# JuliaDSP/DSP.jl

Hardware: AMD Instinct MI355X
Metric: Gsamples/s filt+welch, 1 Gsample Float32 stream; achieved HBM GB/s vs roofline (higher is better)
Workload: dtype f32; 1 GPU; filt(256 taps, overlap-save nfft 2048) + welch_pgram(nfft 4096, hanning, 50 %) per 2^30-sample Float32 stream; one stream per GPU; RCCL all-reduce of the PSD for N>1; samples_per_gpu=1073741824, engine=fused, collective=none (1 GPU), collective_check=not run (--full checks it)

## Files before the change

dsp.jl_amd/_lib.py:

```python
from __future__ import annotations

import ctypes as C
import os
import threading

HERE = os.path.dirname(os.path.abspath(__file__))
LIB_PATH = os.path.join(HERE, "libmi355dsp" + ("_" + os.environ["MDSP_LIB_TAG"] if os.environ.get("MDSP_LIB_TAG") else "") + ".so")

OK, ERR_ARGUMENT, ERR_DOMAIN, ERR_DIMENSION, ERR_ASSERTION, ERR_UNSUPPORTED, ERR_DEVICE, ERR_NOMEM = 0, -1, -2, -3, -4, -5, -6, -7
F32, F64, C32, C64 = 0, 1, 2, 3
ENGINE_AUTO, ENGINE_FUSED, ENGINE_ROCFFT = 0, 1, 2
OLS_FILT, OLS_CONV = 0, 1
HOST_PINNED = 1
COMM_ID_BYTES = 128


class ArgumentError(ValueError):
    """Julia ``ArgumentError``."""


class DomainError(ValueError):
    """Julia ``DomainError``."""


# ... 43 lines not shown
    "mdsp_ols_geometry_for": (ci, [i64, i64, i64, ci, ci, ci, pi64, pi64, pint, pint, pint]),
    "mdsp_ols_exec": (ci, [vp, vp, i64, i64, i64, vp, i64, i64, vp]),
    "mdsp_ols_exec_range": (ci, [vp, vp, i64, i64, i64, vp, i64, i64, i64, vp]),
    "mdsp_ols_exec_host": (ci, [vp, vp, i64, i64, i64, vp, i64, i64, ci]),
    "mdsp_ols_segment": (ci, [vp, vp, i64, i64, i64, vp, vp]),
    "mdsp_frames": (ci, [vp, i64, ci, i64, i64, i64, pdbl, i64, i64, vp, vp]),
    "mdsp_welch_plan_create": (ci, [pvp, i64, i64, i64, pdbl, cd, ci, ci, ci]),
    "mdsp_welch_plan_destroy": (ci, [vp]),
    "mdsp_welch_plan_info": (ci, [vp, pi64, pint]),
    "mdsp_welch_exec": (ci, [vp, vp, i64, i64, i64, vp, i64, vp]),
    "mdsp_welch_reset": (ci, [vp]),
    "mdsp_welch_accumulate": (ci, [vp, vp, i64, i64, i64, vp]),
    "mdsp_welch_frames_accumulated": (ci, [vp, pi64]),
    "mdsp_welch_finalize": (ci, [vp, i64, vp, i64, vp]),
    "mdsp_welch_accumulator": (ci, [vp, pvp, pi64]),
    "mdsp_welch_exec_host": (ci, [vp, vp, i64, i64, i64, vp, i64, ci]),
    "mdsp_comm_unique_id": (ci, [vp]),
    "mdsp_comm_init_rank": (ci, [pvp, vp, ci, ci]),
    "mdsp_comm_destroy": (ci, [vp]),
    "mdsp_comm_info": (ci, [vp, pint, pint]),
    "mdsp_allreduce_sum": (ci, [vp, vp, i64, ci, vp]),
    "mdsp_welch_mean_allreduce": (ci, [vp, vp, i64, i64, i64, vp, vp, vp]),
    "mdsp_welch_allreduce": (ci, [vp, vp, vp]),
    "mdsp_host_alloc": (ci, [pvp, C.c_size_t]),
    "mdsp_host_free": (ci, [vp]),
    "mdsp_host_register": (ci, [vp, C.c_size_t]),
    "mdsp_host_unregister": (ci, [vp]),
    "mdsp_channel_sum": (ci, [vp, i64, i64, i64, ci, vp, vp]),
    "mdsp_stft_plan_create": (ci, [pvp, i64, i64, i64, pdbl, cd, ci, ci, ci, ci]),
    "mdsp_stft_plan_destroy": (ci, [vp]),
# ... 138 lines not shown
```

dsp.jl_amd/csrc/spectral.hip:

```cpp
#include <algorithm>
#include <atomic>
#include <cstdlib>

#include <map>
#include <memory>
#include <mutex>
#include <vector>

#include "common.h"
#include "devio.h"
#include "fft_lds.h"
#include "fft_wg.h"
#include "hostfft.h"
#include "rocfft_wrap.h"
#include "welch_plan.h"
#include "hostpipe.h"
#include "gx_kernels.h"

using namespace mdsp;
using mdsp::fft::cx;

namespace {

inline int64_t rocfft_chunk_bytes() {
// ... 938 lines not shown
            for (int e = 0; e < E; ++e) accp[e] = fft::lanefma(v[e], v[e], accp[e]);
            if (++since == FLUSH) flush();
        } else {
#pragma unroll
            for (int e = 0; e < E; ++e) acc[e] += (double)(v[e].x * v[e].x + v[e].y * v[e].y);
        }
    }
    if constexpr (PAIR) {
        flush();
    } else {
#pragma unroll
        for (int e = 0; e < E; ++e) part[t + T * e] = acc[e];
    }
}

template <int N>
__global__ __launch_bounds__(N / 16, 2) void welch_half3_kernel(SpecArgs a) {
    using R = float;
    constexpr int E = 16, H = 8, PADSHIFT = 5;
    using C = fft::Cfg<N, E>;
    constexpr int T = C::T;
    static_assert(T % 64 == 0 && T >= 128, "one transform per workgroup");
    constexpr int NTWA = C::NTW > 0 ? C::NTW : 1;
    constexpr int REGION = fft::wg_lds_elems<C, PADSHIFT, 1>();
    __shared__ __attribute__((aligned(16))) cx<R> lds[REGION];
    const int t = threadIdx.x;
    const cx<R>* table = static_cast<const cx<R>*>(a.table);
    const int64_t ch = blockIdx.y;

    cx<R> tw[NTWA];
    fft::load_twiddles<C, R, 1, fft::TW_REG>(tw, t, table);
    cx<R> wp[H];
    {
        double wd[E];
        load_window_regs<E, T>(wd, a.win, a.n, t);
#pragma unroll
        for (int e = 0; e < H; ++e) wp[e] = {(R)wd[e], (R)wd[e + H]};
    }
    constexpr int FLUSH = 128;
    cx<R> accp[E];
#pragma unroll
    for (int e = 0; e < E; ++e) accp[e] = {(R)0, (R)0};
    double* part = static_cast<double*>(a.out) + ((int64_t)blockIdx.x * a.nch + ch) * N;
    const __amdgpu_buffer_rsrc_t prs = io::make_rsrc(part, (int64_t)N * 8);
    int since = 0;
    bool first = true;
    auto flush = [&]() {
        int off = t * 8;
        asm volatile("" : "+v"(off));
        if (first) {
#pragma unroll
            for (int e = 0; e < E; ++e) io::Ld<double>::store((double)accp[e].x + (double)accp[e].y, prs, off + T * e * 8);
        } else {
#pragma unroll
            for (int e = 0; e < E; ++e) {
                const double s = io::Ld<double>::load(prs, off + T * e * 8) + ((double)accp[e].x + (double)accp[e].y);
                io::Ld<double>::store(s, prs, off + T * e * 8);
            }
        }
#pragma unroll
        for (int e = 0; e < E; ++e) accp[e] = {(R)0, (R)0};
        first = false;
        since = 0;
    };

    const R* sc = static_cast<const R*>(a.s) + ch * a.lds_;
    const int64_t nslots = (int64_t)gridDim.x;
    int64_t wbase = (int64_t)blockIdx.x * a.run_len, wj = 0;
    auto unit_cur = [&](bool more) { return (more && wbase + wj < a.units_per_ch) ? wbase + wj : a.units_per_ch; };
    auto walk = [&]() {
        if (++wj == a.run_len) {
            wj = 0;
            wbase += nslots * a.run_len;
        }
    };
    auto half_rsrc = [&](int64_t u, int h, bool on) {
        const int64_t pos = u * N + (int64_t)h * (N / 2);
        return io::make_rsrc(sc + pos, on ? std::min<int64_t>(N / 2, a.len - pos) * 4 : 0);
    };
    auto ld8 = [&](cx<R> (&dst)[H], bool to_x, const __amdgpu_buffer_rsrc_t r) {
        int off = t * 4;
        asm volatile("" : "+v"(off));
#pragma unroll
// ... 81 lines not shown
#else
        fft::pass0_windowed<C, PADSHIFT>(Q, F, wp, t, lds);
#endif
        const bool carry = unext == u + 1 && unext < a.units_per_ch;
        load_unit(F, Q, !xa, unext, carry);
        u = unext;
        tail();
    };
    for (int64_t it = 0; it < a.niter; it += 2) {
        unit(P1, P2, true, it + 1 < a.niter);
        if (it + 1 < a.niter) unit(P2, P1, false, it + 2 < a.niter);
    }
    flush();
#ifdef MDSP_WELCH_PROF
    if (a.rinv && (threadIdx.x & 63) == 0) {
        unsigned long long* rec = (unsigned long long*)a.rinv + ((size_t)blockIdx.x * (T / 64) + threadIdx.x / 64) * 16;
        for (int k = 0; k < 13; ++k) rec[k] = prof_sum[k];
        rec[13] = prof_units;
        rec[14] = prof_last - prof_t0;
    }
#undef MDSP_STAMP
#endif
}

template <int N> int welch_run_half3(mdsp_welch_plan_s* pl, SpecArgs& a, hipStream_t st, int* nslices) {
    auto kern = welch_half3_kernel<N>;
    constexpr int threads = N / 16;
    int grid = 1;
    MDSP_TRY(grid_for(kern, threads, a.units_per_ch, a.nch, &grid));
    MDSP_TRY(pl->partial.reserve(sizeof(double) * (size_t)grid * (size_t)a.nch * N));
    a.out = pl->partial.p;
    set_schedule(a, a.units_per_ch, (int64_t)grid);
#ifdef MDSP_WELCH_PROF
    static DevBuf profbuf;
    const size_t nrec = (size_t)grid * (threads / 64);
    MDSP_TRY(profbuf.reserve(nrec * 16 * 8));
    a.rinv = a.nch == 1 ? static_cast<const double*>(profbuf.p) : nullptr;
// ... 19 lines not shown
            totmax = std::max(totmax, (double)h[r * 16 + 14]);
        }
        static const char* nm[13] = {"flush+loop", "load-issue", "barrier1", "reload1", "barrier2", "pass1+ldsW", "barrier3", "reload2", "barrier4", "pass2+acc",
                                     "memwait", "pass0-valu", "pass0-ldsW"};
        fprintf(stderr, "WELCHPROF grid %d x %d waves, %.4f ms, %.0f units/wave, clocks/unit %.0f (max-wave total %.0f clocks -> %.3f GHz):", grid, threads / 64, ms,
                units / nrec, tot / units, totmax, totmax / (ms * 1e6));
        for (int k : {10, 11, 12, 1, 2, 3, 4, 5, 6, 7, 8, 9, 0}) fprintf(stderr, " %s %.0f", nm[k], sum[k] / units);
        fprintf(stderr, "\n");
    }
    (void)hipEventDestroy(e0); (void)hipEventDestroy(e1);
#endif
    *nslices = grid;
    return MDSP_OK;
}

#include "welch_w64.h"

template <typename R, int N, int E, int G, int TWMODE, int PADSHIFT, int NBUF>
int welch_run_half(mdsp_welch_plan_s* pl, SpecArgs& a, hipStream_t st, int* nslices) {
    auto kern = welch_half_kernel<R, N, E, G, TWMODE, PADSHIFT, NBUF>;
    constexpr int threads = (N / E) * G;
    int grid = 1;
    MDSP_TRY(grid_for(kern, threads, cdiv(a.units_per_ch, G), a.nch, &grid));
    MDSP_TRY(pl->partial.reserve(sizeof(double) * (size_t)grid * G * (size_t)a.nch * N));
    a.out = pl->partial.p;
    set_schedule(a, a.units_per_ch, (int64_t)grid * G);
    hipLaunchKernelGGL(kern, dim3(grid, (unsigned)a.nch), dim3(threads), 0, st, a);
    MDSP_LAUNCH_CHECK();
    *nslices = grid * G;
    return MDSP_OK;
// ... 54 lines not shown
    } else {
        bool done = false;
        if constexpr (CPLX && sizeof(R) == 4 && Gm::E > 4) {
            constexpr int T = N / Gm::E;
            const int shift = (!MDSP_DBG(stft_noshift) && a.n == N && a.hop % T == 0 && a.hop / T < Gm::E) ? (int)(a.hop / T) : 0;
            done = shift == 1 || shift == 2 || shift == 4;
            if (shift == 1) rc = welch_run_fused<R, N, Gm::E, Gm::G, Gm::TWREG, pad_default<R>(), CPLX, Gm::NBUF, false, 1>(pl, a, st, &nslices);
            else if (shift == 2) rc = welch_run_fused<R, N, Gm::E, Gm::G, Gm::TWREG, pad_default<R>(), CPLX, Gm::NBUF, false, 2>(pl, a, st, &nslices);
            else if (shift == 4) rc = welch_run_fused<R, N, Gm::E, Gm::G, Gm::TWREG, pad_default<R>(), CPLX, Gm::NBUF, false, 4>(pl, a, st, &nslices);
        }
        if (!done) rc = welch_run_fused<R, N, Gm::E, Gm::G, Gm::TWREG, pad_default<R>(), CPLX, Gm::NBUF, sizeof(R) == 8>(pl, a, st, &nslices);
    }
finalize:
    if (rc != MDSP_OK) return rc;
    MDSP_TRY(pl->reduced.reserve(sizeof(double) * (size_t)a.nch * N));
    MDSP_TRY(reduce_partials(pl, pl->partial.as<double>(), pl->reduced.as<double>(), nslices, a.nch, N, pl->acc_fresh ? 0 : 1, st));
reduced_done:
    if (rc != MDSP_OK) return rc;
    set_fused_sums(pl);
    return MDSP_OK;
}

template <typename R, bool CPLX>
int welch_accumulate_fused(mdsp_welch_plan_s* pl, const void* s, int64_t len, int64_t nch, int64_t lds_, hipStream_t st) {
    const int64_t K = mdsp_frame_count(len, pl->n, pl->noverlap), hop = pl->n - pl->noverlap, N = pl->nfft;
    const double* win = pl->have_win ? pl->win.as<double>() : nullptr;
    if (pl->route != MDSP_ROUTE_POW2 || K == 0) MDSP_TRY(pl->reduced.reserve(sizeof(double) * (size_t)nch * (size_t)N));
    if (K == 0) {
        if (pl->acc_fresh) {
            MDSP_HIP(hipMemsetAsync(pl->reduced.p, 0, sizeof(double) * (size_t)nch * (size_t)N, st));
            set_fused_sums(pl);
// ... 51 lines not shown
            MDSP_TRY(ctcols_welch(pl->ctcols, pl->dtype, s, lds_, K, hop, nch, (int)pl->n, N, pl->r0, win, st, &ngroups, &pl->partial));
            break;
        case MDSP_ROUTE_CTROWS:
            MDSP_TRY(ctrows_welch(pl->ctrows, pl->dtype, pl->r0, s, lds_, K, hop, nch, (int)pl->n, N, win, pl->reduced.as<double>(), pl->acc_fresh, st));
            set_fused_sums(pl);
            return MDSP_OK;
        case MDSP_ROUTE_BIG: {
            using TT = std::conditional_t<CPLX, cx<R>, R>;
            for (int64_t c = 0; c < nch; ++c)
                MDSP_TRY(big::welch(pl->big, pl->dtype, pl->n, N, static_cast<const TT*>(s) + c * lds_, K, hop, win, pl->reduced.as<double>() + c * N, pl->acc_fresh, st));
            set_fused_sums(pl);
            return MDSP_OK;
        }
        default: MDSP_FAIL(MDSP_ERR_ASSERTION, "Welch plan with route %d on the fused engine", pl->route);
    }
    MDSP_TRY(reduce_partials(pl, pl->partial.as<double>(), pl->reduced.as<double>(), (int)ngroups, nch, (int)N, pl->acc_fresh ? 0 : 1, st));
    set_fused_sums(pl);
    return MDSP_OK;
}

}

namespace mdsp {
int gx_run(int id, const GxArgs& a, unsigned grid_x, unsigned grid_y, int threads, size_t lds_bytes, hipStream_t st) {
    switch (id) {
#define MDSP_GX_CASE(ID) case ID: return gx_run_##ID(a, grid_x, grid_y, threads, lds_bytes, st);
        MDSP_GX_CASE(0) MDSP_GX_CASE(1) MDSP_GX_CASE(2) MDSP_GX_CASE(3) MDSP_GX_CASE(5) MDSP_GX_CASE(6) MDSP_GX_CASE(7) MDSP_GX_CASE(8)
        MDSP_GX_CASE(10) MDSP_GX_CASE(11) MDSP_GX_CASE(12) MDSP_GX_CASE(14) MDSP_GX_CASE(15) MDSP_GX_CASE(16) MDSP_GX_CASE(17) MDSP_GX_CASE(19)
#undef MDSP_GX_CASE
        default: MDSP_FAIL(MDSP_ERR_ASSERTION, "gx kernel id %d", id);
    }
// ... 85 lines not shown
    return MDSP_OK;
}

static int welch_check_args(mdsp_welch_plan plan, const void* s_dev, int64_t len, int64_t nch, int64_t lds_) {
    if (!plan) MDSP_FAIL(MDSP_ERR_ARGUMENT, "plan is NULL");
    if (len < 0 || nch < 0) MDSP_FAIL(MDSP_ERR_ARGUMENT, "negative size");
    if (!s_dev && len > 0 && nch > 0) MDSP_FAIL(MDSP_ERR_ARGUMENT, "s is NULL");
    if (nch > 1 && lds_ < len) MDSP_FAIL(MDSP_ERR_DIMENSION, "leading dimension smaller than the column length");
    if (nch > 65535) MDSP_FAIL(MDSP_ERR_UNSUPPORTED, "more than 65535 channels per call");
    return MDSP_OK;
}

int mdsp_welch_reset(mdsp_welch_plan plan) {
    if (!plan) MDSP_FAIL(MDSP_ERR_ARGUMENT, "plan is NULL");
    plan->acc_fresh = true;
    plan->acc_frames = 0;
    plan->acc_nch = 0;
    plan->frames_on_device = false;
    plan->sums_global = false;
    return MDSP_OK;
}

int mdsp_welch_accumulate(mdsp_welch_plan plan, const void* s_dev, int64_t len, int64_t nch, int64_t lds_, void* stream) {
    MDSP_TRY(welch_check_args(plan, s_dev, len, nch, lds_));
    if (nch == 0) return MDSP_OK;
    if (!plan->acc_fresh && plan->acc_nch != nch)
        MDSP_FAIL(MDSP_ERR_DIMENSION, "accumulating %lld channels into sums of %lld channels (mdsp_welch_reset first)", (long long)nch, (long long)plan->acc_nch);
    if (plan->sums_global)
        MDSP_FAIL(MDSP_ERR_ARGUMENT, "these sums are totals over ranks (mdsp_welch_allreduce ran): mdsp_welch_reset before accumulating again");
    hipStream_t st = as_stream(stream);
// ... 21 lines not shown
        MDSP_HIP(hipStreamSynchronize(plan->count_stream));
        MDSP_HIP(hipMemcpy(&k, plan->kdev.p, sizeof(double), hipMemcpyDeviceToHost));
        *frames_per_channel = (int64_t)k;
    }
    return MDSP_OK;
}

int mdsp_welch_accumulator(mdsp_welch_plan plan, void** acc_dev, int64_t* count) {
    if (!plan || !acc_dev || !count) MDSP_FAIL(MDSP_ERR_ARGUMENT, "NULL argument");
    if (plan->acc_fresh) MDSP_FAIL(MDSP_ERR_ARGUMENT, "nothing accumulated since the last mdsp_welch_reset");
    *acc_dev = plan->acc_ptr();
    *count = (int64_t)plan->acc_nslices * plan->acc_nch * plan->acc_nacc;
    return MDSP_OK;
}

int mdsp_welch_finalize(mdsp_welch_plan plan, int64_t frames_total, void* psd_dev, int64_t ldp, void* stream) {
    if (!plan) MDSP_FAIL(MDSP_ERR_ARGUMENT, "plan is NULL");
    if (!psd_dev) MDSP_FAIL(MDSP_ERR_ARGUMENT, "out is NULL");
    if (plan->acc_fresh) MDSP_FAIL(MDSP_ERR_ARGUMENT, "nothing accumulated since the last mdsp_welch_reset");
    if (plan->acc_nch > 1 && ldp < plan->nout) MDSP_FAIL(MDSP_ERR_DIMENSION, "leading dimension smaller than the column length");
    const int64_t K = frames_total > 0 ? frames_total : (plan->frames_on_device ? 0 : plan->acc_frames);
    return dtype_is_double(plan->dtype) ? welch_finalize<double>(plan, K, plan->acc_nch, psd_dev, ldp, as_stream(stream))
                                        : welch_finalize<float>(plan, K, plan->acc_nch, psd_dev, ldp, as_stream(stream));
}

int mdsp_welch_exec(mdsp_welch_plan plan, const void* s_dev, int64_t len, int64_t nch, int64_t lds_, void* psd_dev, int64_t ldp, void* stream) {
    MDSP_TRY(welch_check_args(plan, s_dev, len, nch, lds_));
    if (nch == 0) return MDSP_OK;
    if (!psd_dev) MDSP_FAIL(MDSP_ERR_ARGUMENT, "out is NULL");
    if (nch > 1 && ldp < plan->nout) MDSP_FAIL(MDSP_ERR_DIMENSION, "leading dimension smaller than the column length");
    MDSP_TRY(mdsp_welch_reset(plan));
    MDSP_TRY(mdsp_welch_accumulate(plan, s_dev, len, nch, lds_, stream));
    return mdsp_welch_finalize(plan, 0, psd_dev, ldp, stream);
}

}

template <typename R>
__global__ __launch_bounds__(256) void channel_sum_kernel(const R* __restrict__ psd, R* __restrict__ out, int64_t nout, int64_t nch, int64_t ldp, double scale) {
    const int64_t j = (int64_t)blockIdx.x * blockDim.x + threadIdx.x;
    if (j >= nout) return;
    double a = 0;
    for (int64_t c = 0; c < nch; ++c) a += (double)psd[c * ldp + j];
    const R sum = (R)a;
    out[j] = scale == 1.0 ? sum : (R)((double)sum * scale);
}

// ... 659 lines not shown
```

dsp.jl_amd/csrc/welch_plan.h:

```cpp
#pragma once

#include "common.h"
#include "rocfft_wrap.h"
#include "bigfft.h"
#include "gx_plan.h"
#include "spectral_ctcols.h"
#include "spectral_ctrows.h"

struct mdsp_welch_plan_s {
    int dtype = MDSP_F32, engine = MDSP_ENGINE_ROCFFT, onesided = 1;
    int route = MDSP_ROUTE_ROCFFT, r0 = 0;
    int64_t n = 0, noverlap = 0, nfft = 0, nout = 0;
    double r = 1;
    bool have_win = false;
    mdsp::DevBuf win, table, partial, reduced;
    mdsp::RocPlan fwd;
    mdsp::DevBuf fr, spec;
    int64_t batch = 0;
    int variant = 0;
    bool acc_fresh = true;
    int64_t acc_nch = 0, acc_frames = 0;
    mdsp::DevBuf kdev;
    mdsp::DevBuf redtmp;
    mdsp::big::EngineHolder big;
    mdsp::GxPlan gx;
    mdsp::DevBuf winr;
    bool winr_ready = false;
    mdsp::CtRowsPlan ctrows;
    mdsp::CtColsPlan ctcols;
    mdsp::DevBuf w64prep;
    bool frames_on_device = false;
    bool sums_global = false;
    hipStream_t count_stream = nullptr;
    int acc_nslices = 1, acc_nacc = 0, acc_mode = 0;
    double* acc_ptr() const { return engine == MDSP_ENGINE_ROCFFT ? partial.as<double>() : reduced.as<double>(); }
};
```

dsp.jl_amd/csrc/welch_w64.h:

```cpp
#pragma once

namespace w64 {

constexpr int N = 4096, HALF = N / 2;

#include "welch_w64c_asm_co.h"
#include "welch_w64d_asm_co.h"

struct W64AsmArgs {
    const float* s;
    float* part;
    const float* winpairs;
    const float* tw;
    int64_t lds_, units, run_len, nch;
    int nflush, pad;
};
static_assert(sizeof(W64AsmArgs) == 72, "kernarg layout of mdsp_welch_w64_asm");

__global__ __launch_bounds__(256) void w64asm_prepare_kernel(const double* __restrict__ win, int n, const cx<float>* __restrict__ table, float* __restrict__ out) {
    const int i = blockIdx.x * blockDim.x + threadIdx.x;
    if (i < HALF) {
        out[2 * i] = (float)(i < n ? (win ? win[i] : 1.0) : 0.0);
        out[2 * i + 1] = (float)((i + HALF) < n ? (win ? win[i + HALF] : 1.0) : 0.0);
    }
// ... 7 lines not shown
            tw[14 + 2 * (j - 1) + 1] = b.y;
        }
        for (int k1 = 0; k1 < 4; ++k1) {
            const int m = i + 64 * k1;
            const int e[4] = {m, 2 * m, 4 * m, m + N / 8};
            for (int q = 0; q < 4; ++q) {
                const cx<float> w = table[e[q] & (N - 1)];
                out[2 * HALF + 28 * 64 + 128 * (4 * k1 + q) + 2 * i] = w.x;
                out[2 * HALF + 28 * 64 + 128 * (4 * k1 + q) + 2 * i + 1] = w.y;
            }
        }
    }
}

constexpr int W64_RED_GROUPS = 128;
__global__ __launch_bounds__(256) void w64asm_reduce1_kernel(const float* __restrict__ part, double* __restrict__ tmp, int nslots, int nflush, int64_t nch, int rows_per_group,
                                                             int64_t units, int64_t run_len) {
    const int k4 = (blockIdx.x * 256 + threadIdx.x) * 4;
    const int g = blockIdx.y;
    const int64_t ch = blockIdx.z;
    const int rows = nslots * nflush;
    const int r0 = g * rows_per_group, r1 = min(rows, r0 + rows_per_group);
    double a0 = 0, a1 = 0, a2 = 0, a3 = 0;
#pragma unroll 4
    for (int r = r0; r < r1; ++r) {
        const int sl = r / nflush, f = r - sl * nflush;
        const int64_t mine = min(run_len, units - (int64_t)sl * run_len);
        float4 v = make_float4(0.f, 0.f, 0.f, 0.f);
        if ((int64_t)f * 128 < mine) v = *reinterpret_cast<const float4*>(part + (((int64_t)sl * nch + ch) * nflush + f) * N + k4);
        a0 += (double)v.x;
        a1 += (double)v.y;
        a2 += (double)v.z;
        a3 += (double)v.w;
    }
    double* o = tmp + ((int64_t)ch * W64_RED_GROUPS + g) * N + k4;
    o[0] = a0;
    o[1] = a1;
    o[2] = a2;
    o[3] = a3;
}
__global__ __launch_bounds__(256) void w64asm_reduce2_kernel(const double* __restrict__ tmp, double* __restrict__ reduced, int ngroups, int accumulate) {
    __shared__ double sm[8][32];
    const int b = threadIdx.x & 31, gl = threadIdx.x >> 5;
    const int k = blockIdx.x * 32 + b;
    const int64_t ch = blockIdx.y;
    double t = 0;
    for (int g = gl; g < ngroups; g += 8) t += tmp[((int64_t)ch * W64_RED_GROUPS + g) * N + k];
    sm[gl][b] = t;
    __syncthreads();
    if (gl == 0) {
        t = sm[0][b];
#pragma unroll
        for (int i = 1; i < 8; ++i) t += sm[i][b];
        reduced[ch * N + k] = accumulate ? reduced[ch * N + k] + t : t;
    }
}

struct W64AsmModule {
    hipModule_t mod = nullptr;
    hipFunction_t fn = nullptr;
};
inline int w64asm_function(hipFunction_t* fn, int variant) {
    if (variant != 43 && variant != 44) MDSP_FAIL(MDSP_ERR_ARGUMENT, "no hand-allocated Welch kernel for variant %d", variant);
    static std::mutex mu;
    static W64AsmModule mods[2][64];
    int dev = 0;
    MDSP_HIP(hipGetDevice(&dev));
    std::lock_guard<std::mutex> lk(mu);
    W64AsmModule& m = mods[variant - 43][dev & 63];
    if (!m.fn) {
        MDSP_HIP(hipModuleLoadData(&m.mod, variant == 44 ? welch_w64d_asm_co : welch_w64c_asm_co));
// ... 3 lines not shown
    return MDSP_OK;
}

template <int DUMMY = 0> int welch_run_w64asm(mdsp_welch_plan_s* pl, SpecArgs& a, hipStream_t st, bool* handled, int variant = 44) {
    *handled = false;
    hipFunction_t fn = nullptr;
    MDSP_TRY(w64asm_function(&fn, variant));
    constexpr size_t PREP_FLOATS = 2 * HALF + 28 * 64 + 16 * 128;
    if (pl->w64prep.bytes == 0) {
        MDSP_TRY(pl->w64prep.reserve(PREP_FLOATS * sizeof(float)));
        hipLaunchKernelGGL(w64asm_prepare_kernel, dim3(HALF / 256), dim3(256), 0, st, a.win, a.n, static_cast<const cx<float>*>(a.table), pl->w64prep.as<float>());
        MDSP_LAUNCH_CHECK();
    }
    const int64_t units = a.K / 2;
    MDSP_TRY(pl->reduced.reserve(sizeof(double) * (size_t)a.nch * N));
    bool fresh = pl->acc_fresh;
    if (units > 0) {
        const int64_t per_ch = std::max<int64_t>(1, (int64_t)device_cu_count() / std::max<int64_t>(1, a.nch));
        const int grid = (int)std::max<int64_t>(1, std::min<int64_t>(cdiv(units, 8), per_ch));
        const int64_t nslots = (int64_t)grid * 8;
        const int64_t run_len = cdiv(units, nslots);
        const int nflush = (int)cdiv(run_len, 128);
        const size_t part_bytes = sizeof(float) * (size_t)nslots * (size_t)a.nch * (size_t)nflush * N;
        const size_t tmp_bytes = sizeof(double) * (size_t)a.nch * W64_RED_GROUPS * N;
        MDSP_TRY(pl->partial.reserve(part_bytes + tmp_bytes));
        W64AsmArgs ka;
        ka.s = static_cast<const float*>(a.s);
        ka.part = pl->partial.as<float>();
        ka.winpairs = pl->w64prep.as<float>();
        ka.tw = pl->w64prep.as<float>() + 2 * HALF;
        ka.lds_ = a.lds_;
        ka.units = units;
        ka.run_len = run_len;
        ka.nch = a.nch;
        ka.nflush = nflush;
        ka.pad = 0;
        size_t ksz = sizeof(ka);
        void* cfg[] = {HIP_LAUNCH_PARAM_BUFFER_POINTER, &ka, HIP_LAUNCH_PARAM_BUFFER_SIZE, &ksz, HIP_LAUNCH_PARAM_END};
        MDSP_HIP(hipModuleLaunchKernel(fn, (unsigned)grid, (unsigned)a.nch, 1, 512, 1, 1, 0, st, nullptr, cfg));
        {
            const int rows = (int)nslots * nflush;
            const int rpg = (int)cdiv(rows, W64_RED_GROUPS), ngroups = (int)cdiv(rows, rpg);
            double* tmp = reinterpret_cast<double*>(static_cast<char*>(pl->partial.p) + part_bytes);
            hipLaunchKernelGGL(w64asm_reduce1_kernel, dim3(N / 1024, (unsigned)ngroups, (unsigned)a.nch), dim3(256), 0, st, pl->partial.as<float>(), tmp, (int)nslots, nflush,
                               a.nch, rpg, units, run_len);
            MDSP_LAUNCH_CHECK();
            hipLaunchKernelGGL(w64asm_reduce2_kernel, dim3(N / 32, (unsigned)a.nch), dim3(256), 0, st, tmp, pl->reduced.as<double>(), ngroups, fresh ? 0 : 1);
            MDSP_LAUNCH_CHECK();
        }
        fresh = false;
    }
    if (a.K & 1) {
        SpecArgs t = a;
        t.s = static_cast<const float*>(a.s) + (a.K - 1) * a.hop;
        t.len = a.n;
        t.K = 1;
        t.units_per_ch = 1;
        int ns2 = 0;
        MDSP_TRY((welch_run_half3<N>(pl, t, st, &ns2)));
        hipLaunchKernelGGL(reduce_partials_kernel, dim3((unsigned)cdiv(N, 32), (unsigned)a.nch), dim3(256), 0, st, pl->partial.as<double>(), pl->reduced.as<double>(), ns2,
                           a.nch, N, fresh ? 0 : 1);
        MDSP_LAUNCH_CHECK();
        fresh = false;
    }
    *handled = true;
    return MDSP_OK;
}

}
```

include/mi355dsp.h:

```cpp
#ifndef MI355DSP_H
#define MI355DSP_H

#include <stddef.h>
#include <stdint.h>

#ifdef __cplusplus
extern "C" {
#endif

#define MDSP_VERSION 100

enum {
    MDSP_OK = 0,
    MDSP_ERR_ARGUMENT = -1,
    MDSP_ERR_DOMAIN = -2,
    MDSP_ERR_DIMENSION = -3,
    MDSP_ERR_ASSERTION = -4,
    MDSP_ERR_UNSUPPORTED = -5,
    MDSP_ERR_DEVICE = -6,
    MDSP_ERR_NOMEM = -7
};

enum { MDSP_F32 = 0, MDSP_F64 = 1, MDSP_C32 = 2 , MDSP_C64 = 3  };

// ... 50 lines not shown
                const double* window_host , int64_t first, int64_t count, void* frames_dev,
                void* stream);

typedef struct mdsp_welch_plan_s* mdsp_welch_plan;
int mdsp_welch_plan_create(mdsp_welch_plan* plan, int64_t n, int64_t noverlap, int64_t nfft,
                           const double* window_host, double r, int onesided, int dtype, int engine);
int mdsp_welch_plan_destroy(mdsp_welch_plan plan);
int mdsp_welch_plan_info(mdsp_welch_plan plan, int64_t* nout, int* engine_used);
int mdsp_welch_exec(mdsp_welch_plan plan, const void* s_dev, int64_t len, int64_t nch, int64_t lds,
                    void* psd_dev, int64_t ldp, void* stream);
int mdsp_welch_reset(mdsp_welch_plan plan);
int mdsp_welch_accumulate(mdsp_welch_plan plan, const void* s_dev, int64_t len, int64_t nch, int64_t lds, void* stream);
int mdsp_welch_frames_accumulated(mdsp_welch_plan plan, int64_t* frames_per_channel);
int mdsp_welch_finalize(mdsp_welch_plan plan, int64_t frames_total, void* psd_dev, int64_t ldp, void* stream);
int mdsp_welch_accumulator(mdsp_welch_plan plan, void** acc_dev, int64_t* count);
int mdsp_channel_sum(const void* psd_dev, int64_t nout, int64_t nch, int64_t ldp, int real_dtype, void* sum_dev,
                     void* stream);

#define MDSP_COMM_ID_BYTES 128
typedef struct mdsp_comm_s* mdsp_comm;
int mdsp_comm_unique_id(void* id128 );
int mdsp_comm_init_rank(mdsp_comm* comm, const void* id128, int rank, int nranks);
int mdsp_comm_destroy(mdsp_comm comm);
int mdsp_comm_info(mdsp_comm comm, int* rank, int* nranks);
int mdsp_allreduce_sum(mdsp_comm comm, void* buf_dev, int64_t count, int real_dtype, void* stream);
int mdsp_welch_mean_allreduce(mdsp_welch_plan plan, const void* psd_dev, int64_t nch_local, int64_t ldp, int64_t nch_total,
                              void* mean_dev, mdsp_comm comm, void* stream);
int mdsp_welch_allreduce(mdsp_welch_plan plan, mdsp_comm comm, void* stream);

#define MDSP_HOST_PINNED 1
// ... 148 lines not shown
```

Before: 359.3 Gsamples/s.

## Fuse Welch partial reduction, odd-frame tail and PSD finalize into one kernel

Replaces the two-kernel partial reduction (plus a separate odd-frame half3 launch and reduce) with a single tail kernel. The kernel does a group reduction and uses per-block atomic counters so the last-arriving workgroup performs the final sum and writes the scaled PSD directly. This skips the separate finalize launch when welch_exec is used. The aim is to cut kernel launches and tail latency after the main streaming pass, at the cost of atomic last-block synchronisation and more complex LDS sharing, including running the odd frame inside the tail kernel.

```diff
diff --git a/dsp.jl_amd/_lib.py b/dsp.jl_amd/_lib.py
--- a/dsp.jl_amd/_lib.py
+++ b/dsp.jl_amd/_lib.py
@@ -81,6 +81,7 @@
     "mdsp_welch_frames_accumulated": (ci, [vp, pi64]),
     "mdsp_welch_finalize": (ci, [vp, i64, vp, i64, vp]),
     "mdsp_welch_accumulator": (ci, [vp, pvp, pi64]),
+    "mdsp_welch_rows_reduced": (ci, [vp, pi64]),
     "mdsp_welch_exec_host": (ci, [vp, vp, i64, i64, i64, vp, i64, ci]),
     "mdsp_comm_unique_id": (ci, [vp]),
     "mdsp_comm_init_rank": (ci, [pvp, vp, ci, ci]),
diff --git a/dsp.jl_amd/csrc/spectral.hip b/dsp.jl_amd/csrc/spectral.hip
--- a/dsp.jl_amd/csrc/spectral.hip
+++ b/dsp.jl_amd/csrc/spectral.hip
@@ -976,19 +976,17 @@
     }
 }
 
+template <int N> constexpr int welch_half3_lds() { return fft::wg_lds_elems<fft::Cfg<N, 16>, 5, 1>(); }
 template <int N>
-__global__ __launch_bounds__(N / 16, 2) void welch_half3_kernel(SpecArgs a) {
+__device__ __forceinline__ void welch_half3_units(const SpecArgs& a, cx<float>* lds, const int slot, const int nslots_, const int64_t ch) {
     using R = float;
     constexpr int E = 16, H = 8, PADSHIFT = 5;
     using C = fft::Cfg<N, E>;
     constexpr int T = C::T;
     static_assert(T % 64 == 0 && T >= 128, "one transform per workgroup");
     constexpr int NTWA = C::NTW > 0 ? C::NTW : 1;
-    constexpr int REGION = fft::wg_lds_elems<C, PADSHIFT, 1>();
-    __shared__ __attribute__((aligned(16))) cx<R> lds[REGION];
     const int t = threadIdx.x;
     const cx<R>* table = static_cast<const cx<R>*>(a.table);
-    const int64_t ch = blockIdx.y;
 
     cx<R> tw[NTWA];
     fft::load_twiddles<C, R, 1, fft::TW_REG>(tw, t, table);
@@ -1003,7 +1001,7 @@
     cx<R> accp[E];
 #pragma unroll
     for (int e = 0; e < E; ++e) accp[e] = {(R)0, (R)0};
-    double* part = static_cast<double*>(a.out) + ((int64_t)blockIdx.x * a.nch + ch) * N;
+    double* part = static_cast<double*>(a.out) + ((int64_t)slot * a.nch + ch) * N;
     const __amdgpu_buffer_rsrc_t prs = io::make_rsrc(part, (int64_t)N * 8);
     int since = 0;
     bool first = true;
@@ -1027,8 +1025,8 @@
     };
 
     const R* sc = static_cast<const R*>(a.s) + ch * a.lds_;
-    const int64_t nslots = (int64_t)gridDim.x;
-    int64_t wbase = (int64_t)blockIdx.x * a.run_len, wj = 0;
+    const int64_t nslots = (int64_t)nslots_;
+    int64_t wbase = (int64_t)slot * a.run_len, wj = 0;
     auto unit_cur = [&](bool more) { return (more && wbase + wj < a.units_per_ch) ? wbase + wj : a.units_per_ch; };
     auto walk = [&]() {
         if (++wj == a.run_len) {
@@ -1140,13 +1138,19 @@
     flush();
 #ifdef MDSP_WELCH_PROF
     if (a.rinv && (threadIdx.x & 63) == 0) {
-        unsigned long long* rec = (unsigned long long*)a.rinv + ((size_t)blockIdx.x * (T / 64) + threadIdx.x / 64) * 16;
+        unsigned long long* rec = (unsigned long long*)a.rinv + ((size_t)slot * (T / 64) + threadIdx.x / 64) * 16;
         for (int k = 0; k < 13; ++k) rec[k] = prof_sum[k];
         rec[13] = prof_units;
         rec[14] = prof_last - prof_t0;
     }
 #undef MDSP_STAMP
 #endif
+}
+
+template <int N>
+__global__ __launch_bounds__(N / 16, 2) void welch_half3_kernel(SpecArgs a) {
+    __shared__ __attribute__((aligned(16))) cx<float> lds[welch_half3_lds<N>()];
+    welch_half3_units<N>(a, lds, (int)blockIdx.x, (int)gridDim.x, (int64_t)blockIdx.y);
 }
 
 template <int N> int welch_run_half3(mdsp_welch_plan_s* pl, SpecArgs& a, hipStream_t st, int* nslices) {
@@ -1196,6 +1200,7 @@
     return MDSP_OK;
 }
 
+#include "welch_tail.h"
 #include "welch_w64.h"
 
 template <typename R, int N, int E, int G, int TWMODE, int PADSHIFT, int NBUF>
@@ -1280,7 +1285,9 @@
 finalize:
     if (rc != MDSP_OK) return rc;
     MDSP_TRY(pl->reduced.reserve(sizeof(double) * (size_t)a.nch * N));
-    MDSP_TRY(reduce_partials(pl, pl->partial.as<double>(), pl->reduced.as<double>(), nslices, a.nch, N, pl->acc_fresh ? 0 : 1, st));
+    pl->rows_reduced = nslices;
+    if (pl->fin_psd) MDSP_TRY(tail::run_rows<R>(pl, nslices, a.nch, N, a.K, st));
+    else MDSP_TRY(reduce_partials(pl, pl->partial.as<double>(), pl->reduced.as<double>(), nslices, a.nch, N, pl->acc_fresh ? 0 : 1, st));
 reduced_done:
     if (rc != MDSP_OK) return rc;
     set_fused_sums(pl);
@@ -1362,7 +1369,9 @@
         }
         default: MDSP_FAIL(MDSP_ERR_ASSERTION, "Welch plan with route %d on the fused engine", pl->route);
     }
-    MDSP_TRY(reduce_partials(pl, pl->partial.as<double>(), pl->reduced.as<double>(), (int)ngroups, nch, (int)N, pl->acc_fresh ? 0 : 1, st));
+    pl->rows_reduced = ngroups;
+    if (pl->fin_psd) MDSP_TRY(tail::run_rows<R>(pl, (int)ngroups, nch, (int)N, K, st));
+    else MDSP_TRY(reduce_partials(pl, pl->partial.as<double>(), pl->reduced.as<double>(), (int)ngroups, nch, (int)N, pl->acc_fresh ? 0 : 1, st));
     set_fused_sums(pl);
     return MDSP_OK;
 }
@@ -1478,6 +1487,7 @@
 int mdsp_welch_reset(mdsp_welch_plan plan) {
     if (!plan) MDSP_FAIL(MDSP_ERR_ARGUMENT, "plan is NULL");
     plan->acc_fresh = true;
+    plan->rows_reduced = 0;
     plan->acc_frames = 0;
     plan->acc_nch = 0;
     plan->frames_on_device = false;
@@ -1529,6 +1539,12 @@
     return MDSP_OK;
 }
 
+int mdsp_welch_rows_reduced(mdsp_welch_plan plan, int64_t* rows) {
+    if (!plan || !rows) MDSP_FAIL(MDSP_ERR_ARGUMENT, "NULL argument");
+    *rows = plan->rows_reduced;
+    return MDSP_OK;
+}
+
 int mdsp_welch_finalize(mdsp_welch_plan plan, int64_t frames_total, void* psd_dev, int64_t ldp, void* stream) {
     if (!plan) MDSP_FAIL(MDSP_ERR_ARGUMENT, "plan is NULL");
     if (!psd_dev) MDSP_FAIL(MDSP_ERR_ARGUMENT, "out is NULL");
@@ -1545,7 +1561,12 @@
     if (!psd_dev) MDSP_FAIL(MDSP_ERR_ARGUMENT, "out is NULL");
     if (nch > 1 && ldp < plan->nout) MDSP_FAIL(MDSP_ERR_DIMENSION, "leading dimension smaller than the column length");
     MDSP_TRY(mdsp_welch_reset(plan));
-    MDSP_TRY(mdsp_welch_accumulate(plan, s_dev, len, nch, lds_, stream));
+    plan->fin_psd = plan->engine == MDSP_ENGINE_ROCFFT ? nullptr : psd_dev;
+    plan->fin_ldp = ldp;
+    plan->fin_done = false;
+    const int rc = mdsp_welch_accumulate(plan, s_dev, len, nch, lds_, stream);
+    plan->fin_psd = nullptr;
+    if (rc != MDSP_OK || plan->fin_done) return rc;
     return mdsp_welch_finalize(plan, 0, psd_dev, ldp, stream);
 }
 
diff --git a/dsp.jl_amd/csrc/welch_plan.h b/dsp.jl_amd/csrc/welch_plan.h
--- a/dsp.jl_amd/csrc/welch_plan.h
+++ b/dsp.jl_amd/csrc/welch_plan.h
@@ -28,6 +28,11 @@
     bool winr_ready = false;
     mdsp::CtRowsPlan ctrows;
     mdsp::CtColsPlan ctcols;
+    mdsp::DevBuf tailcnt;
+    void* fin_psd = nullptr;
+    int64_t fin_ldp = 0;
+    bool fin_done = false;
+    int64_t rows_reduced = 0;
     mdsp::DevBuf w64prep;
     bool frames_on_device = false;
     bool sums_global = false;
diff --git a/dsp.jl_amd/csrc/welch_tail.h b/dsp.jl_amd/csrc/welch_tail.h
--- /dev/null
+++ b/dsp.jl_amd/csrc/welch_tail.h
@@ -0,0 +1,279 @@
+#pragma once
+
+namespace tail {
+
+struct TailArgs {
+    const void* rows;
+    double* tmp;
+    double* reduced;
+    const double* odd;
+    void* psd;
+    unsigned* counters;
+    int64_t ldp, nch;
+    int N, nrows, per_group, ngroups;
+    int accumulate, mode, nout, has_odd;
+    double r_total;
+    int nslots, nflush;
+    int64_t units, run_len;
+};
+
+template <int SL> __device__ __forceinline__ int slot_bin(int N, int b, int q) {
+    constexpr int PB = SL / 2;
+    const int p = b * PB + (q < PB ? q : SL - 1 - q);
+    if (p >= (N + 1) / 2) return -1;
+    if (q < PB) return p;
+    if (p == 0) return (N & 1) ? -1 : N / 2;
+    return N - p;
+}
+
+struct __attribute__((packed, aligned(4))) Float4U {
+    float x, y, z, w;
+};
+
+template <int SL> constexpr int lds_sums() { return 8 * SL * 8; }
+template <int SL> constexpr int lds_flags() { return lds_sums<SL>() + SL * 8; }
+constexpr int MAX_FLAGS = 64;
+constexpr int W64_GPW = 4;
+
+template <typename RowT, typename R, int SL>
+__device__ __forceinline__ void phase2(const TailArgs& a, char* smem, const int b, const int NB, const int64_t ch) {
+    constexpr int PB = SL / 2;
+    constexpr bool W64 = sizeof(RowT) == 4;
+    double* sm = reinterpret_cast<double*>(smem);
+    double* fin = reinterpret_cast<double*>(smem + lds_sums<SL>());
+    const int tid = threadIdx.x, N = a.N;
+    const int nsum = a.ngroups > 0 ? a.ngroups : (W64 ? 0 : a.nrows);
+    const double* grp = a.tmp + ((int64_t)ch * NB + b) * a.ngroups * SL;
+    for (int q0 = 0; q0 < SL; q0 += 32) {
+        const int q = q0 + (tid & 31), gl = tid >> 5;
+        const int bin = slot_bin<SL>(N, b, q);
+        double t = 0;
+        if (bin >= 0) {
+            if (a.ngroups > 0) {
+#pragma unroll 4
+                for (int g = gl; g < nsum; g += 8) t += grp[(int64_t)g * SL + q];
+            } else if constexpr (!W64) {
+                const double* rows = static_cast<const double*>(a.rows);
+#pragma unroll 4
+                for (int s = gl; s < nsum; s += 8) t += rows[((int64_t)s * a.nch + ch) * N + bin];
+            }
+        }
+        sm[gl * SL + q] = t;
+    }
+    __syncthreads();
+    if (tid < SL) {
+        const int bin = slot_bin<SL>(N, b, tid);
+        double r = 0;
+        if (bin >= 0) {
+            double t = sm[tid];
+#pragma unroll
+            for (int i = 1; i < 8; ++i) t += sm[i * SL + tid];
+            bool have = false;
+            if (a.accumulate) {
+                r = a.reduced[ch * N + bin];
+                have = true;
+            }
+            if (nsum > 0) {
+                r = have ? r + t : t;
+                have = true;
+            }
+            if (a.has_odd) {
+                const double o = a.odd[ch * N + bin];
+                r = have ? r + o : o;
+            }
+            a.reduced[ch * N + bin] = r;
+        }
+        fin[tid] = r;
+    }
+    __syncthreads();
+    if (a.psd && tid < PB) {
+        const int lo = slot_bin<SL>(N, b, tid), hi = slot_bin<SL>(N, b, SL - 1 - tid);
+        if (lo >= 0) {
+            R* out = static_cast<R*>(a.psd) + ch * a.ldp;
+            const double x = fin[tid], y = fin[SL - 1 - tid];
+            const double m1 = 1.0 / a.r_total, m2 = 2.0 / a.r_total;
+            if (a.mode == 1) {
+                out[lo] = (R)(x * m1);
+                if (hi >= 0) out[hi] = (R)(y * m1);
+            } else if (lo == 0) {
+                out[0] = (R)(0.5 * (x + x) * m1);
+                if (hi >= 0) out[hi] = (R)(0.5 * (y + y) * m1);
+            } else {
+                const double v = 0.5 * (x + y);
+                out[lo] = (R)(v * (a.mode == 3 ? m2 : m1));
+                if (a.mode != 3) out[hi] = (R)(v * m1);
+            }
+        }
+    }
+    __syncthreads();
+}
+
+template <typename RowT, typename R, int SL>
+__global__ __launch_bounds__(256, 2) void welch_tail_kernel(const TailArgs a, const SpecArgs oddu) {
+    constexpr bool W64 = sizeof(RowT) == 4;
+    constexpr int N_W64 = 4096;
+    constexpr int LDS_BYTES = W64 ? (int)sizeof(cx<float>) * welch_half3_lds<N_W64>() : lds_flags<SL>() + 4 * MAX_FLAGS;
+    static_assert(LDS_BYTES >= lds_flags<SL>() + 4 * MAX_FLAGS && (!W64 || W64_GPW * 16 * 32 * 16 <= LDS_BYTES), "one LDS array holds every phase");
+    __shared__ __attribute__((aligned(16))) char smem[LDS_BYTES];
+    int* flags = reinterpret_cast<int*>(smem + lds_flags<SL>());
+    const int tid = threadIdx.x, N = a.N;
+    const int64_t ch = blockIdx.y;
+    const int NB = ((N + 1) / 2 + SL / 2 - 1) / (SL / 2);
+    unsigned* cnt = a.counters + ch * NB;
+    const unsigned expected = (unsigned)((a.ngroups + (W64 ? W64_GPW : 1) - 1) / (W64 ? W64_GPW : 1) + a.has_odd);
+    int w = (int)blockIdx.x;
+
+    if constexpr (W64) {
+        if (a.has_odd && w == 0) {
+            welch_half3_units<N_W64>(oddu, reinterpret_cast<cx<float>*>(smem), 0, 1, ch);
+            asm volatile("s_waitcnt vmcnt(0)" ::: "memory");
+            __syncthreads();
+            if (tid < NB) {
+                __builtin_amdgcn_fence(__ATOMIC_RELEASE, "agent");
+                asm volatile("s_waitcnt vmcnt(0)" ::: "memory");
+                const bool last = __hip_atomic_fetch_add(&cnt[tid], 1u, __ATOMIC_RELAXED, __HIP_MEMORY_SCOPE_AGENT) == expected - 1;
+                if (last) {
+                    __hip_atomic_store(&cnt[tid], 0u, __ATOMIC_RELAXED, __HIP_MEMORY_SCOPE_AGENT);
+                    __builtin_amdgcn_fence(__ATOMIC_ACQUIRE, "agent");
+                    asm volatile("s_waitcnt vmcnt(0)" ::: "memory");
+                }
+                flags[tid] = last;
+            }
+            __syncthreads();
+            for (int b = 0; b < NB; ++b)
+                if (flags[b]) phase2<RowT, R, SL>(a, smem, b, NB, ch);
+            return;
+        }
+        w -= a.has_odd;
+    }
+    if (a.ngroups == 0) {
+        if constexpr (!W64) phase2<RowT, R, SL>(a, smem, w, NB, ch);
+        return;
+    }
+    constexpr int GPW = W64 ? W64_GPW : 1;
+    const int g = (w / NB) * GPW, b = w % NB;
+    double* o = a.tmp + (((int64_t)ch * NB + b) * a.ngroups + g) * SL;
+    if constexpr (W64) {
+        const float* part = static_cast<const float*>(a.rows);
+        float4* stage = reinterpret_cast<float4*>(smem);
+        const int ql = tid & 31, rl = tid >> 5, q = 4 * ql;
+        int bin[4];
+#pragma unroll
+        for (int i = 0; i < 4; ++i) bin[i] = slot_bin<SL>(N, b, q + i);
+        const bool vec = bin[3] == bin[0] + 3;
+        double a0 = 0, a1 = 0, a2 = 0, a3 = 0;
+        for (int roff = 0; roff < a.per_group; roff += 16) {
+#pragma unroll
+            for (int i = 0; i < 2 * GPW; ++i) {
+                const int gg = i >> 1, rg = roff + 8 * (i & 1) + rl;
+                const int row = (g + gg) * a.per_group + rg;
+                const int rowc = min(row, a.nrows - 1);
+                const int sl = rowc / a.nflush, f = rowc - sl * a.nflush;
+                const int64_t mine = min(a.run_len, a.units - (int64_t)sl * a.run_len);
+                const bool counts = rg < a.per_group && row < a.nrows && (int64_t)f * 128 < mine;
+                const float* src = part + (((int64_t)sl * a.nch + ch) * a.nflush + f) * N;
+                float4 v;
+                if (vec) {
+                    const Float4U u = *reinterpret_cast<const Float4U*>(src + bin[0]);
+                    v = make_float4(u.x, u.y, u.z, u.w);
+                } else {
+                    v = make_float4(src[bin[0]], src[bin[1]], src[bin[2]], src[bin[3]]);
+                }
+                stage[(16 * gg + 8 * (i & 1) + rl) * 32 + ql] = counts ? v : make_float4(0.f, 0.f, 0.f, 0.f);
+            }
+            __syncthreads();
+            if (rl < GPW) {
+#pragma unroll
+                for (int i = 0; i < 16; ++i) {
+                    const float4 v = stage[(16 * rl + i) * 32 + ql];
+                    a0 += (double)v.x;
+                    a1 += (double)v.y;
+                    a2 += (double)v.z;
+                    a3 += (double)v.w;
+                }
+            }
+            __syncthreads();
+        }
+        if (rl < GPW && g + rl < a.ngroups) {
+            double* og = o + (int64_t)rl * SL;
+            og[q] = a0;
+            og[q + 1] = a1;
+            og[q + 2] = a2;
+            og[q + 3] = a3;
+        }
+    } else {
+        static_assert(W64 || SL == 256, "one slot per thread");
+        const double* rows = static_cast<const double*>(a.rows);
+        const int bin = slot_bin<SL>(N, b, tid);
+        const int r0 = g * a.per_group, r1 = min(a.nrows, r0 + a.per_group);
+        double s = 0;
+        if (bin >= 0) {
+#pragma unroll 4
+            for (int r = r0; r < r1; ++r) s += rows[((int64_t)r * a.nch + ch) * N + bin];
+        }
+        o[tid] = s;
+    }
+    asm volatile("s_waitcnt vmcnt(0)" ::: "memory");
+    __syncthreads();
+    if (tid == 0) {
+        __builtin_amdgcn_fence(__ATOMIC_RELEASE, "agent");
+        asm volatile("s_waitcnt vmcnt(0)" ::: "memory");
+        const bool last = __hip_atomic_fetch_add(&cnt[b], 1u, __ATOMIC_RELAXED, __HIP_MEMORY_SCOPE_AGENT) == expected - 1;
+        if (last) {
+            __hip_atomic_store(&cnt[b], 0u, __ATOMIC_RELAXED, __HIP_MEMORY_SCOPE_AGENT);
+            __builtin_amdgcn_fence(__ATOMIC_ACQUIRE, "agent");
+            asm volatile("s_waitcnt vmcnt(0)" ::: "memory");
+        }
+        flags[0] = last;
+    }
+    __syncthreads();
+    if (flags[0]) phase2<RowT, R, SL>(a, smem, b, NB, ch);
+}
+
+constexpr int SL_W64 = 128, SL_ROWS = 256;
+inline int blocks_of(int N, int SL) { return (int)cdiv((N + 1) / 2, SL / 2); }
+
+inline int reserve_counters(mdsp_welch_plan_s* pl, size_t count, hipStream_t st) {
+    if (pl->tailcnt.bytes < sizeof(unsigned) * count) {
+        MDSP_TRY(pl->tailcnt.reserve(std::max<size_t>(4096, sizeof(unsigned) * count)));
+        MDSP_HIP(hipMemsetAsync(pl->tailcnt.p, 0, pl->tailcnt.bytes, st));
+    }
+    return MDSP_OK;
+}
+
+inline void set_psd(mdsp_welch_plan_s* pl, TailArgs& t, int64_t K) {
+    t.psd = pl->fin_psd;
+    t.ldp = pl->fin_ldp;
+    t.mode = dtype_is_complex(pl->dtype) ? 1 : (pl->onesided ? 3 : 4);
+    t.nout = (int)pl->nout;
+    t.r_total = (double)K * pl->r;
+    if (pl->fin_psd) pl->fin_done = true;
+}
+
+template <typename R> int run_rows(mdsp_welch_plan_s* pl, int nslices, int64_t nch, int N, int64_t K, hipStream_t st) {
+    constexpr int SL = SL_ROWS;
+    const int NB = blocks_of(N, SL);
+    TailArgs t{};
+    t.rows = pl->partial.p;
+    t.reduced = pl->reduced.as<double>();
+    t.nch = nch;
+    t.N = N;
+    t.nrows = nslices;
+    t.accumulate = pl->acc_fresh ? 0 : 1;
+    unsigned wgs = (unsigned)NB;
+    if (nslices > 2 * REDUCE_GROUPS) {
+        t.per_group = (int)cdiv(nslices, REDUCE_GROUPS);
+        t.ngroups = (int)cdiv(nslices, t.per_group);
+        MDSP_TRY(pl->redtmp.reserve(sizeof(double) * (size_t)nch * NB * t.ngroups * SL));
+        MDSP_TRY(reserve_counters(pl, (size_t)nch * NB, st));
+        t.tmp = pl->redtmp.as<double>();
+        t.counters = pl->tailcnt.as<unsigned>();
+        wgs = (unsigned)(t.ngroups * NB);
+    }
+    set_psd(pl, t, K);
+    hipLaunchKernelGGL((welch_tail_kernel<double, R, SL>), dim3(wgs, (unsigned)nch), dim3(256), 0, st, t, SpecArgs{});
+    MDSP_LAUNCH_CHECK();
+    return MDSP_OK;
+}
+
+}
diff --git a/dsp.jl_amd/csrc/welch_w64.h b/dsp.jl_amd/csrc/welch_w64.h
--- a/dsp.jl_amd/csrc/welch_w64.h
+++ b/dsp.jl_amd/csrc/welch_w64.h
@@ -45,47 +45,6 @@
 }
 
 constexpr int W64_RED_GROUPS = 128;
-__global__ __launch_bounds__(256) void w64asm_reduce1_kernel(const float* __restrict__ part, double* __restrict__ tmp, int nslots, int nflush, int64_t nch, int rows_per_group,
-                                                             int64_t units, int64_t run_len) {
-    const int k4 = (blockIdx.x * 256 + threadIdx.x) * 4;
-    const int g = blockIdx.y;
-    const int64_t ch = blockIdx.z;
-    const int rows = nslots * nflush;
-    const int r0 = g * rows_per_group, r1 = min(rows, r0 + rows_per_group);
-    double a0 = 0, a1 = 0, a2 = 0, a3 = 0;
-#pragma unroll 4
-    for (int r = r0; r < r1; ++r) {
-        const int sl = r / nflush, f = r - sl * nflush;
-        const int64_t mine = min(run_len, units - (int64_t)sl * run_len);
-        float4 v = make_float4(0.f, 0.f, 0.f, 0.f);
-        if ((int64_t)f * 128 < mine) v = *reinterpret_cast<const float4*>(part + (((int64_t)sl * nch + ch) * nflush + f) * N + k4);
-        a0 += (double)v.x;
-        a1 += (double)v.y;
-        a2 += (double)v.z;
-        a3 += (double)v.w;
-    }
-    double* o = tmp + ((int64_t)ch * W64_RED_GROUPS + g) * N + k4;
-    o[0] = a0;
-    o[1] = a1;
-    o[2] = a2;
-    o[3] = a3;
-}
-__global__ __launch_bounds__(256) void w64asm_reduce2_kernel(const double* __restrict__ tmp, double* __restrict__ reduced, int ngroups, int accumulate) {
-    __shared__ double sm[8][32];
-    const int b = threadIdx.x & 31, gl = threadIdx.x >> 5;
-    const int k = blockIdx.x * 32 + b;
-    const int64_t ch = blockIdx.y;
-    double t = 0;
-    for (int g = gl; g < ngroups; g += 8) t += tmp[((int64_t)ch * W64_RED_GROUPS + g) * N + k];
-    sm[gl][b] = t;
-    __syncthreads();
-    if (gl == 0) {
-        t = sm[0][b];
-#pragma unroll
-        for (int i = 1; i < 8; ++i) t += sm[i][b];
-        reduced[ch * N + k] = accumulate ? reduced[ch * N + k] + t : t;
-    }
-}
 
 struct W64AsmModule {
     hipModule_t mod = nullptr;
@@ -119,16 +78,21 @@
     }
     const int64_t units = a.K / 2;
     MDSP_TRY(pl->reduced.reserve(sizeof(double) * (size_t)a.nch * N));
-    bool fresh = pl->acc_fresh;
+    const int64_t per_ch = std::max<int64_t>(1, (int64_t)device_cu_count() / std::max<int64_t>(1, a.nch));
+    const int grid = (int)std::max<int64_t>(1, std::min<int64_t>(cdiv(units, 8), per_ch));
+    const int64_t nslots = units > 0 ? (int64_t)grid * 8 : 0;
+    const int64_t run_len = units > 0 ? cdiv(units, nslots) : 0;
+    const int nflush = units > 0 ? (int)cdiv(run_len, 128) : 1;
+    const int rows = (int)nslots * nflush;
+    const int rpg = (int)cdiv(std::max(rows, 1), W64_RED_GROUPS), ngroups = (int)cdiv(rows, rpg);
+    const size_t part_bytes = sizeof(float) * (size_t)rows * (size_t)a.nch * N;
+    const size_t tmp_bytes = sizeof(double) * (size_t)a.nch * (size_t)ngroups * N;
+    const size_t odd_bytes = (a.K & 1) ? sizeof(double) * (size_t)a.nch * N : 0;
+    MDSP_TRY(pl->partial.reserve(part_bytes + tmp_bytes + odd_bytes));
+    constexpr int NB = N / tail::SL_W64;
+    static_assert(NB <= tail::MAX_FLAGS, "one flag per block of a channel");
+    MDSP_TRY(tail::reserve_counters(pl, (size_t)a.nch * NB, st));
     if (units > 0) {
-        const int64_t per_ch = std::max<int64_t>(1, (int64_t)device_cu_count() / std::max<int64_t>(1, a.nch));
-        const int grid = (int)std::max<int64_t>(1, std::min<int64_t>(cdiv(units, 8), per_ch));
-        const int64_t nslots = (int64_t)grid * 8;
-        const int64_t run_len = cdiv(units, nslots);
-        const int nflush = (int)cdiv(run_len, 128);
-        const size_t part_bytes = sizeof(float) * (size_t)nslots * (size_t)a.nch * (size_t)nflush * N;
-        const size_t tmp_bytes = sizeof(double) * (size_t)a.nch * W64_RED_GROUPS * N;
-        MDSP_TRY(pl->partial.reserve(part_bytes + tmp_bytes));
         W64AsmArgs ka;
         ka.s = static_cast<const float*>(a.s);
         ka.part = pl->partial.as<float>();
@@ -143,31 +107,37 @@
         size_t ksz = sizeof(ka);
         void* cfg[] = {HIP_LAUNCH_PARAM_BUFFER_POINTER, &ka, HIP_LAUNCH_PARAM_BUFFER_SIZE, &ksz, HIP_LAUNCH_PARAM_END};
         MDSP_HIP(hipModuleLaunchKernel(fn, (unsigned)grid, (unsigned)a.nch, 1, 512, 1, 1, 0, st, nullptr, cfg));
-        {
-            const int rows = (int)nslots * nflush;
-            const int rpg = (int)cdiv(rows, W64_RED_GROUPS), ngroups = (int)cdiv(rows, rpg);
-            double* tmp = reinterpret_cast<double*>(static_cast<char*>(pl->partial.p) + part_bytes);
-            hipLaunchKernelGGL(w64asm_reduce1_kernel, dim3(N / 1024, (unsigned)ngroups, (unsigned)a.nch), dim3(256), 0, st, pl->partial.as<float>(), tmp, (int)nslots, nflush,
-                               a.nch, rpg, units, run_len);
-            MDSP_LAUNCH_CHECK();
-            hipLaunchKernelGGL(w64asm_reduce2_kernel, dim3(N / 32, (unsigned)a.nch), dim3(256), 0, st, tmp, pl->reduced.as<double>(), ngroups, fresh ? 0 : 1);
-            MDSP_LAUNCH_CHECK();
-        }
-        fresh = false;
     }
+    tail::TailArgs t{};
+    t.rows = pl->partial.p;
+    t.tmp = reinterpret_cast<double*>(static_cast<char*>(pl->partial.p) + part_bytes);
+    t.reduced = pl->reduced.as<double>();
+    t.counters = pl->tailcnt.as<unsigned>();
+    t.nch = a.nch;
+    t.N = N;
+    t.nrows = rows;
+    t.per_group = rpg;
+    t.ngroups = ngroups;
+    t.accumulate = pl->acc_fresh ? 0 : 1;
+    t.nslots = (int)nslots;
+    t.nflush = nflush;
+    t.units = units;
+    t.run_len = run_len;
+    SpecArgs u = a;
     if (a.K & 1) {
-        SpecArgs t = a;
-        t.s = static_cast<const float*>(a.s) + (a.K - 1) * a.hop;
-        t.len = a.n;
-        t.K = 1;
-        t.units_per_ch = 1;
-        int ns2 = 0;
-        MDSP_TRY((welch_run_half3<N>(pl, t, st, &ns2)));
-        hipLaunchKernelGGL(reduce_partials_kernel, dim3((unsigned)cdiv(N, 32), (unsigned)a.nch), dim3(256), 0, st, pl->partial.as<double>(), pl->reduced.as<double>(), ns2,
-                           a.nch, N, fresh ? 0 : 1);
-        MDSP_LAUNCH_CHECK();
-        fresh = false;
+        t.has_odd = 1;
+        t.odd = reinterpret_cast<double*>(static_cast<char*>(pl->partial.p) + part_bytes + tmp_bytes);
+        u.s = static_cast<const float*>(a.s) + (a.K - 1) * a.hop;
+        u.len = a.n;
+        u.K = 1;
+        u.units_per_ch = 1;
+        u.out = const_cast<double*>(t.odd);
+        set_schedule(u, 1, 1);
     }
+    pl->rows_reduced = rows;
+    tail::set_psd(pl, t, a.K);
+    hipLaunchKernelGGL((tail::welch_tail_kernel<float, float, tail::SL_W64>), dim3((unsigned)(cdiv(ngroups, tail::W64_GPW) * NB + t.has_odd), (unsigned)a.nch), dim3(256), 0, st, t, u);
+    MDSP_LAUNCH_CHECK();
     *handled = true;
     return MDSP_OK;
 }
diff --git a/include/mi355dsp.h b/include/mi355dsp.h
--- a/include/mi355dsp.h
+++ b/include/mi355dsp.h
@@ -88,6 +88,7 @@
 int mdsp_welch_frames_accumulated(mdsp_welch_plan plan, int64_t* frames_per_channel);
 int mdsp_welch_finalize(mdsp_welch_plan plan, int64_t frames_total, void* psd_dev, int64_t ldp, void* stream);
 int mdsp_welch_accumulator(mdsp_welch_plan plan, void** acc_dev, int64_t* count);
+int mdsp_welch_rows_reduced(mdsp_welch_plan plan, int64_t* rows);
 int mdsp_channel_sum(const void* psd_dev, int64_t nout, int64_t nch, int64_t ldp, int real_dtype, void* sum_dev,
                      void* stream);
 
```

Measured after the change: 355.9 Gsamples/s. Within noise of the previous version (-0.9%).
